# MarkTakken/kf2vecFSW

Measured on AMD Instinct MI355X. Metric: Gbases/s k-mer→.kf build at k=7; achieved HBM GB/s vs gfx950 peak, higher is better.
Workload: dtype u32

## Files before the change

include/kf2vec_gpu.h:

```cpp
#ifndef KF2VEC_GPU_H
#define KF2VEC_GPU_H

#include <stddef.h>
#include <stdint.h>

#ifdef __cplusplus
extern "C" {
#endif

#define KF_ABI_VERSION 1

#define KF_OK 0
#define KF_EINVAL (-1)
#define KF_EHIP (-2)
#define KF_ERANGE (-3)
#define KF_EFORMAT (-4)

#define KF_MIN_K 2
#define KF_MAX_K 12
#define KF_SPARSE_MAX_K 31

#define KF_ACCUMULATE 1u

#define KF_FMT_AUTO 0
// ... 12 lines not shown
int kf_index_records(const uint8_t* bytes, uint64_t len, int fmt, uint64_t base,
                     uint64_t* out_iv, uint64_t cap_pairs, uint64_t* n_pairs,
                     int* fmt_detected);

int kf_read_files(const char* const* paths, int32_t n, const uint64_t* sizes, const uint64_t* off,
                  uint8_t* dst, uint64_t piece, int n_threads);

int kf_index_fasta(const uint8_t* d_bytes, const uint64_t* d_goff, int32_t n_genomes,
                   uint64_t batch_bytes, uint64_t* d_excl, uint64_t cap_pairs,
                   uint64_t* d_n_pairs, uint32_t* d_scratch, uint64_t scratch_words, void* stream);

int kf_count_batch(const uint8_t* d_bytes, const uint64_t* d_goff, int32_t n_genomes,
                   const uint64_t* d_excl, uint64_t n_excl,
                   const uint32_t* d_code2col, const uint32_t* d_col2rep, int k,
                   uint32_t* d_counts, uint64_t* d_totals, uint32_t flags, void* stream);

int kf_workspace_reserve(int k, int32_t max_genomes);

int kf_count_launch_info(int k, int* grid, int* block, int* lds_bytes);

uint64_t kf_sparse_workspace_bytes(int k, uint64_t batch_bytes, int32_t n_genomes);
int kf_sparse_count(const uint8_t* d_bytes, const uint64_t* d_goff, int32_t n_genomes,
                    uint64_t batch_bytes, const uint64_t* d_excl, uint64_t n_excl, int k,
                    void* d_work, uint64_t work_bytes, uint64_t* d_keys, uint32_t* d_counts,
                    uint64_t* d_nuniq, void* stream);

const char* kf_build_id(void);

int kf_stream_probe(const uint8_t* d_bytes, uint64_t n, uint32_t* d_out, void* stream);

// ... 46 lines not shown
```

kf2vecfsw_amd/_native.py:

```python
from __future__ import annotations

import ctypes
import os

_HERE = os.path.dirname(os.path.abspath(__file__))
LIB_PATH = os.environ.get("KF2VEC_GPU_LIB") or os.path.join(_HERE, "libkf2vec_gpu.so")

KF_OK = 0
KF_EINVAL = -1
KF_EHIP = -2
KF_ERANGE = -3
KF_EFORMAT = -4
KF_MIN_K = 2
KF_MAX_K = 12
KF_SPARSE_MAX_K = 31
KF_ACCUMULATE = 1
KF_FMT_AUTO, KF_FMT_FASTA, KF_FMT_FASTQ = 0, 1, 2

_u64, _u32, _i32, _i64, _int = ctypes.c_uint64, ctypes.c_uint32, ctypes.c_int32, ctypes.c_int64, ctypes.c_int
_vp, _cp = ctypes.c_void_p, ctypes.c_char_p
_P64 = ctypes.POINTER(ctypes.c_uint64)
_PI = ctypes.POINTER(ctypes.c_int)
SIGNATURES = {
    "kf_abi_version": (_int, []),
    "kf_last_error": (_cp, []),
    "kf_num_bins": (_u64, [_int]),
    "kf_tables": (_int, [_int, _vp, _vp, _P64]),
    "kf_vocab_text": (_int, [_int, _vp, _u64, _P64]),
    "kf_index_records": (_int, [_vp, _u64, _int, _u64, _vp, _u64, _P64, _PI]),
    "kf_count_batch": (_int, [_vp, _vp, _i32, _vp, _u64, _vp, _vp, _int, _vp, _vp, _u32, _vp]),
    "kf_count_launch_info": (_int, [_int, _PI, _PI, _PI]),
    "kf_workspace_release": (_int, []),
    "kf_workspace_reserve": (_int, [_int, _i32]),
    "kf_build_id": (_cp, []),
    "kf_stream_probe": (_int, [_vp, _u64, _vp, _vp]),
    "kf_synth_fasta": (_int, [_vp, _vp, _i32, _i64, _i64, _u64, _u64, _int, _u64, _vp]),
    "kf_synth_genome_bytes": (_u64, [_i64, _u64, _int, _u64]),
    "kf_synth_header_len": (_u64, [_i64]),
    "kf_format_kf": (_int, [_cp, _vp, _u64, _int, _int, _vp, _u64, _P64]),
    "kf_write_kf_files": (_int, [_cp, ctypes.POINTER(_cp), _i32, _vp, _u64, _int, _int, _int]),
    "kf_write_kf_rows": (_int, [_cp, ctypes.POINTER(_cp), _i32, _vp, _u64, _int, _int, _int]),
    "kf_write_kf_segments": (_int, [_i32, ctypes.POINTER(_cp), _vp, _vp, ctypes.POINTER(_cp), ctypes.POINTER(_cp),
                                    _vp, _vp, _u32, _vp, _u64, _int, _int, _int]),
    "kf_write_kf_segments16": (_int, [_i32, ctypes.POINTER(_cp), _vp, _vp, ctypes.POINTER(_cp), ctypes.POINTER(_cp),
                                      _vp, _vp, _u32, _vp, _u64, _int, _int, _int]),
# ... 51 lines not shown
```

kf2vecfsw_amd/counter.py:

```python
from __future__ import annotations

import ctypes
import dataclasses
import os
from typing import Sequence

import numpy as np
import torch

from . import _native as N

ALIGN = 16


def num_bins(k: int) -> int:
    return int(N.lib().kf_num_bins(k))


def tables(k: int) -> tuple[np.ndarray, np.ndarray]:
    nb = num_bins(k)
    code2col = np.empty(1 << (2 * k), dtype=np.uint32)
    col2rep = np.empty(nb, dtype=np.uint32)
    n = ctypes.c_uint64(0)
    N.check(N.lib().kf_tables(k, code2col.ctypes.data, col2rep.ctypes.data, ctypes.byref(n)), "kf_tables")
# ... 153 lines not shown
                    raise N.NativeError(f"short read on {p}")
                got += r
        finally:
            os.close(fd)

    with ThreadPoolExecutor(max_workers=max(1, int(threads))) as ex:
        list(ex.map(read, jobs))
        excl = None
        if index:
            parts = list(ex.map(lambda i: index_records(d[int(off[i]): int(off[i]) + sizes[i]], N.KF_FMT_FASTA,
                                                        int(off[i]))[0], range(len(ranges))))
            excl = (np.concatenate(parts) if parts else np.zeros(0, np.uint64)).astype(np.uint64)
    return HostBatch(data, off, excl, list(names) if names else [f"{p}:{a}" for p, a, _ in ranges])


@dataclasses.dataclass
class DeviceBatch:
    data: torch.Tensor
    off: torch.Tensor
    excl: torch.Tensor
    n: int
    n_excl: int


def index_on_device(data: torch.Tensor, off: torch.Tensor, n: int, nbytes: int) -> tuple[torch.Tensor, int]:
    dev = data.device
    s = _stream_ptr(dev)
    nb = (nbytes + 4095) // 4096
    scratch = torch.empty(nb + 1, dtype=torch.int32, device=dev)
    npairs = torch.zeros(1, dtype=torch.int64, device=dev)
    cap = 64 * n + 4096
    while True:
        excl = torch.empty(max(2 * cap, 2), dtype=torch.int64, device=dev)
        N.check(N.lib().kf_index_fasta(data.data_ptr(), off.data_ptr(), n, nbytes, excl.data_ptr(), cap,
                                       npairs.data_ptr(), scratch.data_ptr(), nb + 1, s), "kf_index_fasta")
        m = int(npairs.item())
        if m <= cap:
            return excl[: 2 * m], m
        cap = m


def to_device(hb: HostBatch, device: torch.device | str = "cuda") -> DeviceBatch:
    dev = torch.device(device)
    if hb.dev_data is not None:
        cur = torch.cuda.current_stream(dev)
        if hb.dev_event is not None:
            cur.wait_event(hb.dev_event)
        data = hb.dev_data
        data.record_stream(cur)
    else:
        data = hb.data.to(dev, non_blocking=True)
    if hb.excl is None:
        pin = hb.data is None or hb.data.is_pinned()
        off = torch.from_numpy(hb.off.view(np.int64))
        off = (off.pin_memory() if pin else off).to(dev, non_blocking=pin)
        with torch.cuda.device(dev):
            excl, m = index_on_device(data, off, hb.n, int(hb.off[-1]))
        return DeviceBatch(data, off, excl if m else torch.zeros(2, dtype=torch.int64, device=dev), hb.n, m)
    ex = hb.excl if hb.excl.size else np.zeros(2, np.uint64)
    pin = hb.data is None or hb.data.is_pinned()
    n_off = (hb.off.size + 1) & ~1
    host = np.zeros(n_off + ex.size, np.int64)
    host[: hb.off.size] = hb.off.view(np.int64)
    host[n_off:] = ex.view(np.int64)
    small = torch.from_numpy(host)
    if pin:
        small = small.pin_memory()
    small = small.to(dev, non_blocking=pin)
    off, excl = small[: hb.off.size], small[n_off:]
    return DeviceBatch(data, off, excl, hb.n, hb.excl.size // 2)


def _stream_ptr(device: torch.device) -> int:
# ... 1 lines not shown


_DEV_TABLES: dict = {}


class KmerCounter:

    def __init__(self, k: int, device: torch.device | str = "cuda"):
        if not (N.KF_MIN_K <= k <= N.KF_MAX_K):
            raise ValueError(f"k={k} out of range [{N.KF_MIN_K}, {N.KF_MAX_K}]")
        self.k = k
        self.device = torch.device(device)
        if self.device.type != "cuda" or not torch.cuda.is_available():
            raise N.NativeError("KmerCounter needs a ROCm GPU (no CPU fallback)")
        self.nbins = num_bins(k)
        key = (k, self.device.index if self.device.index is not None else torch.cuda.current_device())
        if key not in _DEV_TABLES:
            c2c, c2r = tables(k)
            _DEV_TABLES[key] = (torch.from_numpy(c2c.view(np.int32)).to(self.device),
                                torch.from_numpy(c2r.view(np.int32)).to(self.device))
        self.code2col, self.col2rep = _DEV_TABLES[key]

    def launch_info(self) -> tuple[int, int, int]:
        g, b, l = ctypes.c_int(), ctypes.c_int(), ctypes.c_int()
        with torch.cuda.device(self.device):
            N.check(N.lib().kf_count_launch_info(self.k, ctypes.byref(g), ctypes.byref(b), ctypes.byref(l)),
                    "kf_count_launch_info")
        return g.value, b.value, l.value

    def reserve(self, max_genomes: int) -> None:
        with torch.cuda.device(self.device):
            N.check(N.lib().kf_workspace_reserve(self.k, int(max_genomes)), "kf_workspace_reserve")

    def alloc_out(self, n: int) -> tuple[torch.Tensor, torch.Tensor]:
        return (torch.empty((n, self.nbins), dtype=torch.int32, device=self.device),
                torch.empty(n, dtype=torch.int64, device=self.device))

    def count(self, db: DeviceBatch, counts: torch.Tensor | None = None, totals: torch.Tensor | None = None,
              accumulate: bool = False, stream: int | None = None) -> tuple[torch.Tensor, torch.Tensor]:
        if counts is None or totals is None:
            counts, totals = self.alloc_out(db.n)
        assert counts.shape == (db.n, self.nbins) and counts.dtype == torch.int32 and counts.is_contiguous()
        assert totals.shape == (db.n,) and totals.dtype == torch.int64
        assert db.data.data_ptr() % 16 == 0
        s = _stream_ptr(self.device) if stream is None else stream
        with torch.cuda.device(self.device):
            N.check(N.lib().kf_count_batch(
                db.data.data_ptr(), db.off.data_ptr(), db.n, db.excl.data_ptr() if db.n_excl else None,
                db.n_excl, self.code2col.data_ptr(), self.col2rep.data_ptr(), self.k,
                counts.data_ptr(), totals.data_ptr(), N.KF_ACCUMULATE if accumulate else 0, s), "kf_count_batch")
        return counts, totals


class SparseCounter:

    def __init__(self, k: int, device: torch.device | str = "cuda"):
        if not (N.KF_MIN_K <= k <= N.KF_SPARSE_MAX_K):
            raise ValueError(f"k={k} out of range [{N.KF_MIN_K}, {N.KF_SPARSE_MAX_K}]")
        self.k = k
        self.device = torch.device(device)
        if self.device.type != "cuda" or not torch.cuda.is_available():
            raise N.NativeError("SparseCounter needs a ROCm GPU (no CPU fallback)")
        self._work = None

    def workspace_bytes(self, batch_bytes: int, n: int) -> int:
# ... 104 lines not shown
```

kf2vecfsw_amd/csrc/kf_count.hip:

```cpp
#include <hip/hip_runtime.h>
#include <stdint.h>
#include <stdlib.h>

#include <mutex>

#include "kf_front.h"
#include "kf_internal.h"

namespace kf {

constexpr int kBlock = 1024;
#ifndef KF_WAVE_WEIGHTS
#define KF_WAVE_WEIGHTS (20u | 17u << 8 | 11u << 16 | 6u << 24)
#endif
constexpr uint32_t kWaveWeights = KF_WAVE_WEIGHTS;
constexpr int kXRing = 2;

__device__ __forceinline__ uint32_t lds_add_rtn(uint32_t a, uint32_t v) {
    return __hip_atomic_fetch_add((lds_u32*)(uintptr_t)a, v, __ATOMIC_RELAXED, __HIP_MEMORY_SCOPE_WORKGROUP);
}

__device__ __forceinline__ void lds_barrier() { asm volatile("s_waitcnt lgkmcnt(0)\n\ts_barrier" ::: "memory"); }

__device__ __forceinline__ void wg_span(const CountArgs& A, uint64_t& lo, uint64_t& hi) {
// ... 315 lines not shown
            uint32_t r[16];
            xc_wins8(*xs[i], r);
#pragma unroll
            for (int j = 0; j < 16; j += 4) o |= r[j] | r[j + 1] | r[j + 2] | r[j + 3];
        }
    }
    lane_total -= x0.nl + x1.nl + x2.nl;
    carry = tail_pack((uint32_t)__builtin_amdgcn_readlane((int)x2.c, kWave - 1) & TM, 31u, 31u);
    if (__builtin_amdgcn_ballot_w64((o & HOT) != 0) != 0) {
        x_scan_drain<K>(A.code2col, gcounts, lane);
        drained = 1;
    }
    return true;
}

template <int K, bool MASKED>
__device__ __forceinline__ uint32_t x_singles(const uint4 d, const CountArgs& A, uint64_t chunk, int lane,
                                              const ChunkMask& m, uint64_t iv0, uint32_t carry, uint32_t* gcounts,
                                              uint32_t& lane_total, uint32_t& drained) {
    constexpr uint32_t HOT = x_hot<K>();
    uint32_t C, V, EN, ne, own;
    front_end<K, MASKED, false>(d, A, chunk, lane, m, iv0, C, V, EN, ne, own);
    const Windows win = windows<K, MASKED>(C, V, EN, ne, carry, lane);
    const uint32_t wlo = win.wlo, whi = win.whi, R = win.R;
    if constexpr (K == 9) {
        drained |= k9b_region<false>(wlo, whi, R, A, gcounts);
        lane_total += (uint32_t)__builtin_popcount(R);
        return win.next;
    }
    const uint32_t wv[4] = {wlo, __builtin_amdgcn_alignbit(whi, wlo, 8), __builtin_amdgcn_alignbit(whi, wlo, 16),
                            __builtin_amdgcn_alignbit(whi, wlo, 24)};
    uint32_t o = 0;
#pragma unroll
    for (int r = 0; r < 16; ++r) {
        const int fo = (2 * r) & ~7;
        const uint32_t y = __builtin_amdgcn_ubfe(wv[fo >> 3], 2 * r - fo, 2 * K);
        o |= lds_add_rtn((K == 8 ? 0u : XL<K>::P) + ((y >> 1) << 2), ((R >> r) & 1u) * half_one(y));
    }
    if (__builtin_amdgcn_ballot_w64((o & HOT) != 0) != 0) {
        x_scan_drain<K>(A.code2col, gcounts, lane);
        drained = 1;
    }
    lane_total += (uint32_t)__builtin_popcount(R);
    return win.next;
}

template <int K>
__device__ __forceinline__ uint32_t x_range(const CountArgs& A, int32_t g, uint64_t glo, uint64_t ghi, uint64_t lo,
                                            uint64_t hi, int lane, uint32_t& drained) {
    if (lo >= hi) return 0;
    uint32_t* gcounts = A.counts + (uint64_t)g * A.nbins;
    Range rg;
    rg.init(glo, ghi, lo, hi);
    auto load = [&](uint32_t r) {
        return xc_load(A.bytes, rg.c0, r, rg.end_r, lane);
    };
    static_assert(kXRing == 2, "two-deep register ring");
    XBlock buf[K == 9 ? 1 : kXRing];
    XBlock b0, b1;
    if constexpr (K == 9) {
        b0 = load(0);
        b1 = load(kXChunk);
    } else {
#pragma unroll
        for (int j = 0; j < kXRing; ++j) buf[j] = load(j * kXChunk);
    }
    const uint32_t nx = (rg.nch + 2) / 3;
    rg.warm16<K>(A, lane);
    __builtin_amdgcn_s_setprio(0);
    uint32_t carry = rg.carry;
    uint32_t rel = 0;
    const ChunkMask m = rg.mask();
    uint32_t lane_total = 0;
    uint32_t nfast = 0;
    auto step = [&](const XBlock& bf) {
        bool fast = !rg.masked_span(A, rel, kXChunk);
        if (fast)
            fast = xc_fast<K>(bf, A, lane, carry, gcounts, lane_total, drained);
        nfast += fast ? 1u : 0u;
        if (!fast) {
            const bool m0 = rg.masked(A, rel);
            const uint64_t iv0 = rg.iv;
            const bool m1 = rg.masked(A, rel + kChunk);
            const uint64_t iv1 = rg.iv;
            const bool m2 = rg.masked(A, rel + 2 * kChunk);
#pragma unroll
            for (int h = 0; h < 3; ++h) {
                const uint32_t r = rel + h * kChunk;
                if (h > 0 && r >= rg.nch * kChunk) break;
                const bool mh = h == 0 ? m0 : (h == 1 ? m1 : m2);
                const uint64_t ivh = h == 0 ? iv0 : (h == 1 ? iv1 : rg.iv);
                const uint4 hb = bf.q[h];
                if (mh)
                    carry = x_singles<K, true>(hb, A, rg.c0 + r, lane, m, ivh, carry, gcounts, lane_total, drained);
                else
// ... 11 lines not shown
        }
        if (nx & 1u) step(b0);
    } else {
        for (uint32_t i = 0; i + kXRing <= nx; i += kXRing) {
#pragma unroll
            for (int j = 0; j < kXRing; ++j) {
                step(buf[j]);
                buf[j] = load(rel + (kXRing - 1) * kXChunk);
            }
        }
        const uint32_t rem = nx % kXRing;
#pragma unroll
        for (int j = 0; j < kXRing - 1; ++j)
            if (rem > (uint32_t)j) step(buf[j]);
    }
    return lane_total + 48u * nfast;
}

__device__ __forceinline__ uint32_t f_swz(uint32_t y) { return y ^ (((y >> 8) & 15u) << 1); }
__device__ __forceinline__ uint32_t u16sum2(uint32_t w) { return (w & 0xFFFFu) + (w >> 16); }

__device__ __forceinline__ void pair_f_sums(const uint32_t* hist, int tid, uint32_t (&F)[16]) {
    const uint4* h4 = (const uint4*)hist;
#pragma unroll
    for (int i = 0; i < 8; ++i) {
        const uint4 w = h4[i * 1024 + tid];
        F[2 * i] = u16sum2(w.x) + u16sum2(w.y);
        F[2 * i + 1] = u16sum2(w.z) + u16sum2(w.w);
#pragma unroll
        for (int a = 0; a < 4; ++a) {
// ... 11 lines not shown
#pragma unroll
    for (uint32_t m = 0; m < NM; ++m) {
        const uint32_t y = (uint32_t)tid + kBlock * m;
        F[m] = 0;
        if (y < NY) {
            const uint32_t sh = (y & 1u) << 4;
            uint32_t f = u16sum2(hist[2 * y]) + u16sum2(hist[2 * y + 1]);
#pragma unroll
            for (uint32_t a = 0; a < 4; ++a) f += (hist[a * (NY / 2) + (y >> 1)] >> sh) & 0xFFFFu;
            f += (hist[XL<K>::P / 4 + (y >> 1)] >> sh) & 0xFFFFu;
            F[m] = f;
        }
    }
}

template <int K>
__global__ void __launch_bounds__(kBlock) __attribute__((amdgpu_waves_per_eu(4, 4))) k1x_kernel(CountArgs A) {
    static_assert(K >= 2 && K <= 9, "K1x serves k = 2 .. 9 (k = 9: K9b byte counters)");
    extern __shared__ __attribute__((aligned(16))) uint32_t hist[];
    const int tid = threadIdx.x;
    const int lane = tid & (kWave - 1);
    const int wave = __builtin_amdgcn_readfirstlane(tid >> 6);
    {
        uint4* h4 = (uint4*)hist;
        for (uint32_t i = tid; i < XL<K>::bytes / 16; i += kBlock) h4[i] = make_uint4(0u, 0u, 0u, 0u);
    }
    __syncthreads();
    if ((uint32_t)(uintptr_t)(lds_u32*)hist != 0u) __builtin_trap();
    uint64_t span_lo, span_hi;
    wg_span(A, span_lo, span_hi);
    if (span_lo >= span_hi) return;
    int32_t g = (int32_t)wave_upper_bound((uint64_t)A.n_genomes, span_lo, lane,
                                          [&](uint64_t i) { return A.goff[i + 1]; });
    const uint32_t fr_lo = wave_frac((uint32_t)wave, kWaveWeights), fr_hi = wave_frac((uint32_t)wave + 1, kWaveWeights);
    for (; g < A.n_genomes; ++g) {
        __builtin_amdgcn_s_setprio(3);
        const uint64_t glo = A.goff[g], ghi = A.goff[g + 1];
        if (glo >= span_hi) break;
        const uint64_t plo = max(glo, span_lo), phi = min(ghi, span_hi);
        if (phi <= plo) continue;
        const uint64_t lo = split_at_frac(plo, phi, fr_lo), hi = split_at_frac(plo, phi, fr_hi);
        uint32_t drained = 0;
        unsigned long long s = x_range<K>(A, g, glo, ghi, lo, hi, lane, drained);
        uint32_t* gc = A.counts + (uint64_t)g * A.nbins;
        const bool whole = plo == glo && phi == ghi && !(A.flags & KF_ACCUMULATE);
        if constexpr (K == 9) {
            lds_barrier();
            if (lane == 0) hist[XL<K>::P / 4 + wave] = drained;
            lds_barrier();
            const uint4* fl = (const uint4*)(hist + XL<K>::P / 4);
            const uint4 f0 = fl[0], f1 = fl[1], f2 = fl[2], f3 = fl[3];
            const bool any_fix = (f0.x | f0.y | f0.z | f0.w | f1.x | f1.y | f1.z | f1.w | f2.x | f2.y | f2.z |
                                  f2.w | f3.x | f3.y | f3.z | f3.w) != 0;
            const uint8_t* hb = (const uint8_t*)hist;
            for (uint32_t c0 = (uint32_t)tid; c0 < (1u << 17); c0 += 4 * kBlock) {
                uint32_t rep[4];
#pragma unroll
                for (int j = 0; j < 4; ++j) rep[j] = A.col2rep[c0 + j * kBlock];
// ... 232 lines not shown
#pragma unroll
        for (int k = 0; k < 4; ++k)
#pragma unroll
            for (int q = 0; q < 3; ++q) acc ^= v[k][q].x ^ v[k][q].y ^ v[k][q].z ^ v[k][q].w;
    }
    acc = wave_xor(acc);
    if (lane == 0 && acc) atomicXor(out, acc);
}

}

using namespace kf;

namespace {

void* kernel_for(int k) {
    switch (k) {
    case 2: return (void*)&k1x_kernel<2>;
    case 3: return (void*)&k1x_kernel<3>;
    case 4: return (void*)&k1x_kernel<4>;
    case 5: return (void*)&k1x_kernel<5>;
    case 6: return (void*)&k1x_kernel<6>;
    case 7: return (void*)&k1x_kernel<7>;
    case 8: return (void*)&k1x_kernel<8>;
    case 9: return (void*)&k1x_kernel<9>;
    default: return nullptr;
    }
}

int lds_bytes_for(int k) {
    switch (k) {
    case 2: return (int)XL<2>::bytes;
    case 3: return (int)XL<3>::bytes;
    case 4: return (int)XL<4>::bytes;
    case 5: return (int)XL<5>::bytes;
    case 6: return (int)XL<6>::bytes;
    case 7: return (int)XL<7>::bytes;
    case 8: return (int)XL<8>::bytes;
    default: return (int)XL<9>::bytes;
    }
}


int g_grid[KF_MAX_K + 1][64];
std::mutex g_grid_mu;

int launch_info(int k, int* grid, int* block, int* lds) {
    int dev = 0;
    if (hipGetDevice(&dev) != hipSuccess) return kf_fail(KF_EHIP, "hipGetDevice failed");
    if (dev < 0 || dev >= 64) return kf_fail(KF_EINVAL, "device index out of range");
    const int l = lds_bytes_for(k);
    std::lock_guard<std::mutex> lk(g_grid_mu);
    int& gr = g_grid[k][dev];
    if (!gr) {
        void* fn = kernel_for(k);
        if (hipFuncSetAttribute(fn, hipFuncAttributeMaxDynamicSharedMemorySize, l) != hipSuccess)
            return kf_fail(KF_EHIP, "hipFuncSetAttribute(MaxDynamicSharedMemorySize) failed");
        int per_cu = 0, cus = 0;
        if (hipOccupancyMaxActiveBlocksPerMultiprocessor(&per_cu, fn, kBlock, l) != hipSuccess)
            return kf_fail(KF_EHIP, "hipOccupancyMaxActiveBlocksPerMultiprocessor failed");
        if (hipDeviceGetAttribute(&cus, hipDeviceAttributeMultiprocessorCount, dev) != hipSuccess)
            return kf_fail(KF_EHIP, "hipDeviceGetAttribute(MultiprocessorCount) failed");
        gr = (per_cu < 1 ? 1 : per_cu) * (cus > 0 ? cus : 1);
    }
    *grid = gr;
    *block = kBlock;
    *lds = l;
    return KF_OK;
}
}

extern "C" int kf_count_launch_info(int k, int* grid, int* block, int* lds_bytes) {
    if (k < KF_MIN_K || k > KF_MAX_K) return kf_fail(KF_EINVAL, "k out of range [2, 12]");
    if (!grid || !block || !lds_bytes) return kf_fail(KF_EINVAL, "null output pointer");
    if (k >= 10) return bucket_launch_info(k, grid, block, lds_bytes);
    return launch_info(k, grid, block, lds_bytes);
}

extern "C" int kf_workspace_reserve(int k, int32_t max_genomes) {
    if (k < KF_MIN_K || k > KF_MAX_K) return kf_fail(KF_EINVAL, "k out of range [2, 12]");
    if (max_genomes < 0) return kf_fail(KF_EINVAL, "max_genomes < 0");
    if (k >= 10) return bucket_reserve(k, max_genomes);
    int grid = 0, block = 0, lds = 0;
    return launch_info(k, &grid, &block, &lds);
}

extern "C" int kf_count_batch(const uint8_t* d_bytes, const uint64_t* d_goff, int32_t n_genomes,
                              const uint64_t* d_excl, uint64_t n_excl, const uint32_t* d_code2col,
                              const uint32_t* d_col2rep, int k, uint32_t* d_counts, uint64_t* d_totals,
                              uint32_t flags, void* stream) {
    if (k < KF_MIN_K || k > KF_MAX_K) return kf_fail(KF_EINVAL, "k out of range [2, 12]");
    if (n_genomes < 0) return kf_fail(KF_EINVAL, "n_genomes < 0");
    if (n_genomes == 0) return KF_OK;
    if (!d_bytes || !d_goff || !d_counts || !d_totals || !d_code2col || !d_col2rep)
        return kf_fail(KF_EINVAL, "null device pointer");
    if (n_excl && !d_excl) return kf_fail(KF_EINVAL, "d_excl is null but n_excl > 0");
    if (((uintptr_t)d_bytes) & 15) return kf_fail(KF_EINVAL, "d_bytes must be 16-byte aligned");
    const uint64_t nb = kf_num_bins(k);
    hipStream_t s = (hipStream_t)stream;
// ... 7 lines not shown
            hipMemsetAsync(d_totals, 0, (size_t)n_genomes * sizeof(uint64_t), s) != hipSuccess)
            return kf_fail(KF_EHIP, "hipMemsetAsync failed");
    }
    CountArgs A;
    A.bytes = d_bytes;
    A.goff = d_goff;
    A.excl = d_excl;
    A.n_excl = n_excl;
    A.code2col = d_code2col;
    A.col2rep = d_col2rep;
    A.counts = d_counts;
    A.totals = (unsigned long long*)d_totals;
    A.nbins = (uint32_t)nb;
    A.n_genomes = n_genomes;
    A.flags = flags;
    if (bucket) return bucket_launch(A, k, flags, s);
    int grid = 0, block = 0, lds = 0;
    const int rc = launch_info(k, &grid, &block, &lds);
    if (rc) return rc;

    void* args[] = {&A};
    if (hipLaunchKernel(kernel_for(k), dim3(grid), dim3(block), args, (size_t)lds, s) != hipSuccess)
        return kf_fail(KF_EHIP, "count kernel launch failed: %s", hipGetErrorString(hipGetLastError()));
    return KF_OK;
}

extern "C" int kf_stream_probe(const uint8_t* d_bytes, uint64_t n, uint32_t* d_out, void* stream) {
    if (!d_bytes || !d_out) return kf_fail(KF_EINVAL, "null device pointer");
    if (((uintptr_t)d_bytes) & 15) return kf_fail(KF_EINVAL, "d_bytes must be 16-byte aligned");
    if (n == 0) return KF_OK;
    int dev = 0, cus = 0;
    if (hipGetDevice(&dev) != hipSuccess ||
        hipDeviceGetAttribute(&cus, hipDeviceAttributeMultiprocessorCount, dev) != hipSuccess)
        return kf_fail(KF_EHIP, "device query failed");
    hipLaunchKernelGGL(stream_probe_kernel, dim3(2 * (cus > 0 ? cus : 1)), dim3(1024), 0, (hipStream_t)stream, d_bytes,
                       n, d_out);
    if (hipGetLastError() != hipSuccess) return kf_fail(KF_EHIP, "stream probe launch failed");
// ... 17 lines not shown
```

kf2vecfsw_amd/csrc/kf_front.h:

```cpp
#pragma once
#include <hip/hip_runtime.h>
#include <stdint.h>

namespace kf {

constexpr int kWave = 64;
constexpr int kChunk = 1024;

struct CountArgs {
    const uint8_t* bytes;
    const uint64_t* goff;
    const uint64_t* excl;
    uint64_t n_excl;
    const uint32_t* code2col;
    const uint32_t* col2rep;
    uint32_t* counts;
    unsigned long long* totals;
    uint32_t nbins;
    int32_t n_genomes;
    uint32_t flags;
};

__device__ __forceinline__ uint32_t tail_pack(uint32_t codes, uint32_t n, uint32_t ne) {
    return codes | (min(n, 31u) << 22) | (min(ne, 31u) << 27);
}
__device__ __forceinline__ uint32_t t_codes(uint32_t t) { return t & 0x3FFFFFu; }
__device__ __forceinline__ uint32_t t_n(uint32_t t) { return (t >> 22) & 31u; }
__device__ __forceinline__ uint32_t t_ne(uint32_t t) { return t >> 27; }

template <int K>
__device__ __forceinline__ uint32_t tail_combine(uint32_t a, uint32_t b) {
    constexpr uint32_t TM = (K > 1) ? ((1u << (2 * (K - 1))) - 1u) : 0u;
    const uint32_t bn = t_n(b), bne = t_ne(b);
    const uint32_t n = (bn < bne) ? bn : min(t_n(a) + bn, 31u);
    const uint32_t codes =
// ... 230 lines not shown
    uint32_t v = own;
#pragma unroll
    for (int dd = 1; dd < kWave; dd <<= 1) {
        const uint32_t o = __shfl_up(v, dd, kWave);
        if (lane >= dd) v = tail_combine<K>(o, v);
    }
    return (uint32_t)__builtin_amdgcn_readlane((int)v, kWave - 1);
}

template <int K>
__device__ __forceinline__ uint32_t chunk_tail(const uint8_t* bytes, const uint64_t* excl, uint64_t n_excl, int64_t p,
                                               uint64_t glo, int lane) {
    return chunk_tail_data<K>(chunk_tail_load(bytes, p, glo, lane), bytes, excl, n_excl, p, glo, lane);
}


struct Range {
    uint64_t c0, glo, ghi, lo, hi;
    uint32_t lo_r, hi_r, end_r, nch;
    uint64_t iv;
    uint32_t ivs_r, ive_r;
    uint64_t ivs_a, ive_a;
    uint32_t carry;

    __device__ __forceinline__ uint32_t rel_of(uint64_t x) const {
        return x <= c0 ? 0u : (x - c0 >= 0xFFFFFFFFull ? 0xFFFFFFFFu : (uint32_t)(x - c0));
    }
    __device__ __forceinline__ void init(uint64_t glo_, uint64_t ghi_, uint64_t lo_, uint64_t hi_) {
        glo = glo_, ghi = ghi_, lo = lo_, hi = hi_;
        c0 = lo & ~(uint64_t)15;
// ... 161 lines not shown
```

kf2vecfsw_amd/main.py:

```python
from __future__ import annotations

import argparse
import ctypes
import multiprocessing as mp
import os
import sys
from concurrent.futures import ThreadPoolExecutor

import numpy as np

from . import _native as N

__version__ = "kf2vec 0.1.3 (kf2vecfsw_amd MI355X)"

default_k_len = 7
min_k_len = 2
max_k_len = 31
supported_k = range(3, 12)

FORMATS = [".fq", ".fastq", ".fa", ".fna", ".fasta"]
_SUFFIXES = tuple(FORMATS)


def list_inputs(input_dir: str) -> tuple[list[str], list[str]]:
# ... 190 lines not shown
    if not os.path.exists(args.output_dir):
        print("No such directory '{}'".format(args.output_dir), file=sys.stderr)
        sys.exit(0)

    files_names, samples_names = list_inputs(args.input_dir)
    if shard is not None:
        sizes = [os.path.getsize(os.path.join(args.input_dir, f)) for f in files_names]
        mine = shard_files(sizes, samples_names, shard[1])[shard[0]]
        files_names = [files_names[i] for i in mine]
        samples_names = [samples_names[i] for i in mine]
    if args.k not in supported_k:
        raise ValueError("k={} has no vocabulary: supported k are {}..{}".format(
            args.k, supported_k.start, supported_k.stop - 1))

    import torch
    from .counter import KmerCounter, pack_files, to_device

    if shard is not None and not os.environ.get("KF_SHARD"):
        _join_group()
    dflt = f"cuda:{os.environ.get('LOCAL_RANK', '0')}" if shard is not None else "cuda"
    device = torch.device(getattr(args, "device", None) or dflt)
    if not files_names:
        _finish(args, shard, lead)
        return
    counter = KmerCounter(args.k, device)
    paths = [os.path.join(args.input_dir, f) for f in files_names]
    batch_gb = getattr(args, "batch_gb", None)
    fsz = [os.path.getsize(p) for p in paths]
    asz = [(x + 15) // 16 * 16 for x in fsz]
    batches = _size_batches(fsz, _pipeline_budget(paths, batch_gb, fsz), ramp=True,
                            max_files=_count_cap(4 * counter.nbins, batch_gb))
# ... 38 lines not shown
    writer = ThreadPoolExecutor(max_workers=1)
    ahead = n_slots
    reads = deque(reader.submit(pack, i, batches[i]) for i in range(min(ahead, len(batches))))
    big = slot_bytes
    with torch.cuda.stream(copy_stream):
        warm = torch.empty(big + 16, dtype=torch.uint8, device=device)
        warm[:16].zero_()
        del warm
    with torch.cuda.stream(stream):
        torch.cuda.Event(enable_timing=True).record(stream)
    copy_stream.synchronize()
    stream.synchronize()
    writes = []
    behind = max(1, int(os.environ.get("KF_WRITE_BEHIND", "2")))

    def write(ev, host, names):
        ev.synchronize()
        t0 = now_ms()
        c = host.numpy().view(np.uint32)
        write_kf_files(args.output_dir, names, c, args.pseudocount, args.raw_cnt, threads)
        if trace:
            tr.append(("write", names[0] if names else "", t0, now_ms()))

    evs = []
    for bi, idx in enumerate(batches):
        t_wait = now_ms()
        hb = reads.popleft().result()
        if trace:
            tr.append(("got", bi, t_wait, now_ms()))
        if bi + ahead < len(batches):
            reads.append(reader.submit(pack, bi + ahead, batches[bi + ahead]))
        with torch.cuda.stream(stream):
            if trace:
                e = [torch.cuda.Event(enable_timing=True) for _ in range(4)]
                e[0].record(stream)
                evs.append((bi, now_ms(), e))
            db = to_device(hb, device)
            del hb
            if trace:
                e[1].record(stream)
                th = [now_ms()]
            counts, _ = counter.count(db, stream=stream.cuda_stream)
            if trace:
                e[2].record(stream)
                th.append(now_ms())
            keep = [j for j, i in enumerate(idx) if last[samples_names[i]] == i]
            rows = counts if len(keep) == len(idx) else counts[torch.tensor(keep, device=device)]
            host = torch.empty(rows.shape, dtype=rows.dtype, pin_memory=True)
            if trace:
                th.append(now_ms())
            host.copy_(rows, non_blocking=True)
            ev = torch.cuda.Event()
            ev.record(stream)
            if trace:
                e[3].record(stream)
                th.append(now_ms())
        for i in idx:
            if args.pseudocount:
                print(">>> Adding pseudocounts. Sample: {}".format(files_names[i]))
            if not args.raw_cnt:
                print(">>> Normalizing. Sample: {}".format(files_names[i]))
        if bi >= behind:
            writes[bi - behind].result()
        writes.append(writer.submit(write, ev, host, [samples_names[idx[j]] for j in keep]))
        del host, rows, counts, db
        if trace:
            th.append(now_ms())
            tr.append(("issue", bi, th))
    for w in writes:
        w.result()
    t_written = now_ms()
    reader.shutdown()
    writer.shutdown()
    files_pool.shutdown()
    if trace and evs:
        base_cpu = evs[0][1]
        e00 = evs[0][2][0]
        for bi, t_issue, e in evs:
            d = [round(base_cpu + e00.elapsed_time(x), 3) for x in e]
# ... 550 lines not shown
```

Measured before the change: 5751.

## Fuse FASTA header detection into the k-mer count kernel for k up to 9

After: 5752, median of 3. About the same (+0.0%).

```diff
diff --git a/include/kf2vec_gpu.h b/include/kf2vec_gpu.h
--- a/include/kf2vec_gpu.h
+++ b/include/kf2vec_gpu.h
@@ -50,6 +50,11 @@
                    const uint64_t* d_excl, uint64_t n_excl,
                    const uint32_t* d_code2col, const uint32_t* d_col2rep, int k,
                    uint32_t* d_counts, uint64_t* d_totals, uint32_t flags, void* stream);
+
+int kf_count_batch_fasta(const uint8_t* d_bytes, const uint64_t* d_goff, int32_t n_genomes,
+                         const uint32_t* d_code2col, const uint32_t* d_col2rep, int k,
+                         uint32_t* d_counts, uint64_t* d_totals, uint32_t* d_status,
+                         uint32_t flags, void* stream);
 
 int kf_workspace_reserve(int k, int32_t max_genomes);
 
diff --git a/kf2vecfsw_amd/_native.py b/kf2vecfsw_amd/_native.py
--- a/kf2vecfsw_amd/_native.py
+++ b/kf2vecfsw_amd/_native.py
@@ -29,6 +29,7 @@
     "kf_vocab_text": (_int, [_int, _vp, _u64, _P64]),
     "kf_index_records": (_int, [_vp, _u64, _int, _u64, _vp, _u64, _P64, _PI]),
     "kf_count_batch": (_int, [_vp, _vp, _i32, _vp, _u64, _vp, _vp, _int, _vp, _vp, _u32, _vp]),
+    "kf_count_batch_fasta": (_int, [_vp, _vp, _i32, _vp, _vp, _int, _vp, _vp, _vp, _u32, _vp]),
     "kf_count_launch_info": (_int, [_int, _PI, _PI, _PI]),
     "kf_workspace_release": (_int, []),
     "kf_workspace_reserve": (_int, [_int, _i32]),
diff --git a/kf2vecfsw_amd/counter.py b/kf2vecfsw_amd/counter.py
--- a/kf2vecfsw_amd/counter.py
+++ b/kf2vecfsw_amd/counter.py
@@ -191,13 +191,18 @@
     return HostBatch(data, off, excl, list(names) if names else [f"{p}:{a}" for p, a, _ in ranges])
 
 
+FUSED_MAX_K = 9
+
+
 @dataclasses.dataclass
 class DeviceBatch:
     data: torch.Tensor
     off: torch.Tensor
-    excl: torch.Tensor
+    excl: torch.Tensor | None
     n: int
     n_excl: int
+    indexed: bool = True
+    nbytes: int = 0
 
 
 def index_on_device(data: torch.Tensor, off: torch.Tensor, n: int, nbytes: int) -> tuple[torch.Tensor, int]:
@@ -217,7 +222,17 @@
         cap = m
 
 
-def to_device(hb: HostBatch, device: torch.device | str = "cuda") -> DeviceBatch:
+def index_batch(db: DeviceBatch) -> DeviceBatch:
+    if db.indexed:
+        return db
+    dev = db.data.device
+    with torch.cuda.device(dev):
+        excl, m = index_on_device(db.data, db.off, db.n, db.nbytes)
+    return DeviceBatch(db.data, db.off, excl if m else torch.zeros(2, dtype=torch.int64, device=dev), db.n, m,
+                       True, db.nbytes)
+
+
+def to_device(hb: HostBatch, device: torch.device | str = "cuda", index: bool = True) -> DeviceBatch:
     dev = torch.device(device)
     if hb.dev_data is not None:
         cur = torch.cuda.current_stream(dev)
@@ -231,9 +246,8 @@
         pin = hb.data is None or hb.data.is_pinned()
         off = torch.from_numpy(hb.off.view(np.int64))
         off = (off.pin_memory() if pin else off).to(dev, non_blocking=pin)
-        with torch.cuda.device(dev):
-            excl, m = index_on_device(data, off, hb.n, int(hb.off[-1]))
-        return DeviceBatch(data, off, excl if m else torch.zeros(2, dtype=torch.int64, device=dev), hb.n, m)
+        db = DeviceBatch(data, off, None, hb.n, 0, False, int(hb.off[-1]))
+        return index_batch(db) if index else db
     ex = hb.excl if hb.excl.size else np.zeros(2, np.uint64)
     pin = hb.data is None or hb.data.is_pinned()
     n_off = (hb.off.size + 1) & ~1
@@ -265,7 +279,8 @@
         if self.device.type != "cuda" or not torch.cuda.is_available():
             raise N.NativeError("KmerCounter needs a ROCm GPU (no CPU fallback)")
         self.nbins = num_bins(k)
-        key = (k, self.device.index if self.device.index is not None else torch.cuda.current_device())
+        self.status = None
+        key =(k, self.device.index if self.device.index is not None else torch.cuda.current_device())
         if key not in _DEV_TABLES:
             c2c, c2r = tables(k)
             _DEV_TABLES[key] = (torch.from_numpy(c2c.view(np.int32)).to(self.device),
@@ -288,7 +303,17 @@
                 torch.empty(n, dtype=torch.int64, device=self.device))
 
     def count(self, db: DeviceBatch, counts: torch.Tensor | None = None, totals: torch.Tensor | None = None,
-              accumulate: bool = False, stream: int | None = None) -> tuple[torch.Tensor, torch.Tensor]:
+              accumulate: bool = False, stream: int | None = None,
+              status: torch.Tensor | None = None) -> tuple[torch.Tensor, torch.Tensor]:
+        self.status = None
+        if not db.indexed:
+            if self.k > FUSED_MAX_K:
+                db = index_batch(db)
+            else:
+                return self._count_fused(db, counts, totals, accumulate, stream, status)
+        return self._count_indexed(db, counts, totals, accumulate, stream)
+
+    def _count_indexed(self, db, counts=None, totals=None, accumulate=False, stream=None):
         if counts is None or totals is None:
             counts, totals = self.alloc_out(db.n)
         assert counts.shape == (db.n, self.nbins) and counts.dtype == torch.int32 and counts.is_contiguous()
@@ -300,6 +325,35 @@
                 db.data.data_ptr(), db.off.data_ptr(), db.n, db.excl.data_ptr() if db.n_excl else None,
                 db.n_excl, self.code2col.data_ptr(), self.col2rep.data_ptr(), self.k,
                 counts.data_ptr(), totals.data_ptr(), N.KF_ACCUMULATE if accumulate else 0, s), "kf_count_batch")
+        return counts, totals
+
+    def recount_indexed(self, db: DeviceBatch) -> tuple[torch.Tensor, torch.Tensor]:
+        return self._count_indexed(index_batch(db))
+
+    def _count_fused(self, db, counts, totals, accumulate, stream, status):
+        if counts is None or totals is None:
+            counts = torch.empty((db.n, self.nbins), dtype=torch.int32, device=self.device)
+            tot = torch.empty(db.n + 1, dtype=torch.int64, device=self.device)
+            totals, status = tot[: db.n], tot[db.n:].view(torch.int32)[:1]
+        elif status is None:
+            status = torch.zeros(1, dtype=torch.int32, device=self.device)
+        assert counts.shape == (db.n, self.nbins) and counts.dtype == torch.int32 and counts.is_contiguous()
+        assert totals.shape == (db.n,) and totals.dtype == torch.int64
+        assert status.shape == (1,) and status.dtype == torch.int32
+        assert db.data.data_ptr() % 16 == 0
+        s = _stream_ptr(self.device) if stream is None else stream
+        with torch.cuda.device(self.device):
+            N.check(N.lib().kf_count_batch_fasta(
+                db.data.data_ptr(), db.off.data_ptr(), db.n, self.code2col.data_ptr(), self.col2rep.data_ptr(),
+                self.k, counts.data_ptr(), totals.data_ptr(), status.data_ptr(),
+                N.KF_ACCUMULATE if accumulate else 0, s), "kf_count_batch_fasta")
+        self.status = status
+        return counts, totals
+
+    def count_checked(self, db: DeviceBatch) -> tuple[torch.Tensor, torch.Tensor]:
+        counts, totals = self.count(db)
+        if self.status is not None and int(self.status.item()) != 0:
+            counts, totals = self.recount_indexed(db)
         return counts, totals
 
 
diff --git a/kf2vecfsw_amd/csrc/kf_count.hip b/kf2vecfsw_amd/csrc/kf_count.hip
--- a/kf2vecfsw_amd/csrc/kf_count.hip
+++ b/kf2vecfsw_amd/csrc/kf_count.hip
@@ -353,13 +353,25 @@
     return true;
 }
 
-template <int K, bool MASKED>
+template <int K, bool MASKED, bool HDR = false>
 __device__ __forceinline__ uint32_t x_singles(const uint4 d, const CountArgs& A, uint64_t chunk, int lane,
                                               const ChunkMask& m, uint64_t iv0, uint32_t carry, uint32_t* gcounts,
-                                              uint32_t& lane_total, uint32_t& drained) {
+                                              uint32_t& lane_total, uint32_t& drained, uint32_t hm = 0) {
     constexpr uint32_t HOT = x_hot<K>();
     uint32_t C, V, EN, ne, own;
-    front_end<K, MASKED, false>(d, A, chunk, lane, m, iv0, C, V, EN, ne, own);
+    if constexpr (HDR) {
+        static_assert(MASKED, "the header-aware chunk is always masked");
+        uint32_t INV, NNL;
+        classify16(d, C, INV, NNL);
+        const int64_t b0 = (int64_t)(chunk + 16u * (uint32_t)lane);
+        INV |= range_bits(-1, (int64_t)m.glo - b0) | hm;
+        EN = range_bits((int64_t)m.lo - b0, (int64_t)m.hi - b0);
+        V = ~INV & 0xFFFFu;
+        ne = (uint32_t)__builtin_popcount(NNL);
+        compact<true>(NNL ^ 0xFFFFu, C, V, EN);
+    } else {
+        front_end<K, MASKED, false>(d, A, chunk, lane, m, iv0, C, V, EN, ne, own);
+    }
     const Windows win = windows<K, MASKED>(C, V, EN, ne, carry, lane);
     const uint32_t wlo = win.wlo, whi = win.whi, R = win.R;
     if constexpr (K == 9) {
@@ -384,7 +396,7 @@
     return win.next;
 }
 
-template <int K>
+template <int K, bool HDR>
 __device__ __forceinline__ uint32_t x_range(const CountArgs& A, int32_t g, uint64_t glo, uint64_t ghi, uint64_t lo,
                                             uint64_t hi, int lane, uint32_t& drained) {
     if (lo >= hi) return 0;
@@ -405,7 +417,16 @@
         for (int j = 0; j < kXRing; ++j) buf[j] = load(j * kXChunk);
     }
     const uint32_t nx = (rg.nch + 2) / 3;
-    rg.warm16<K>(A, lane);
+    HdrState hs{0u, 0u, 0ull};
+    uint32_t longh = 0;
+    (void)hs, (void)longh;
+    if constexpr (HDR) {
+        const HdrWarm hw = hdr_warm<K>(A.bytes, rg.c0, glo, ghi, lane);
+        rg.carry = rfl(hw.carry);
+        hs = hdr_state(hw.st.in_hdr, hw.st.pnl, (uint32_t)hw.st.hstart, (uint32_t)(hw.st.hstart >> 32));
+    } else {
+        rg.warm16<K>(A, lane);
+    }
     __builtin_amdgcn_s_setprio(0);
     uint32_t carry = rg.carry;
     uint32_t rel = 0;
@@ -413,11 +434,31 @@
     uint32_t lane_total = 0;
     uint32_t nfast = 0;
     auto step = [&](const XBlock& bf) {
-        bool fast = !rg.masked_span(A, rel, kXChunk);
+        bool fast;
+        if constexpr (HDR)
+            fast = !hs.in_hdr && !(rel < rg.lo_r || rel + kXChunk > rg.hi_r);
+        else
+            fast = !rg.masked_span(A, rel, kXChunk);
         if (fast)
             fast = xc_fast<K>(bf, A, lane, carry, gcounts, lane_total, drained);
         nfast += fast ? 1u : 0u;
-        if (!fast) {
+        if constexpr (HDR) {
+            if (fast) {
+                hs.pnl = ((uint32_t)__builtin_amdgcn_readlane((int)bf.q[2].w, kWave - 1) >> 24) == (uint32_t)'\n';
+            } else {
+#pragma unroll
+                for (int h = 0; h < 3; ++h) {
+                    const uint32_t r = rel + h * kChunk;
+                    if (h > 0 && r >= rg.nch * kChunk) break;
+                    const HdrChunk hc =
+                        hdr_chunk(bf.q[h], (int64_t)(rg.c0 + r), glo, ghi, lane, hs.in_hdr, hs.pnl, hs.hstart);
+                    carry = x_singles<K, true, true>(bf.q[h], A, rg.c0 + r, lane, m, 0, carry, gcounts, lane_total,
+                                                     drained, hc.H);
+                    hs = hc.state();
+                    longh |= rfl(hc.longh);
+                }
+            }
+        } else if (!fast) {
             const bool m0 = rg.masked(A, rel);
             const uint64_t iv0 = rg.iv;
             const bool m1 = rg.masked(A, rel + kChunk);
@@ -459,6 +500,9 @@
         for (int j = 0; j < kXRing - 1; ++j)
             if (rem > (uint32_t)j) step(buf[j]);
     }
+    if constexpr (HDR) {
+        if (longh && lane == 0) atomicOr(A.status, 1u);
+    }
     return lane_total + 48u * nfast;
 }
 
@@ -500,7 +544,7 @@
     }
 }
 
-template <int K>
+template <int K, bool HDR = false>
 __global__ void __launch_bounds__(kBlock) __attribute__((amdgpu_waves_per_eu(4, 4))) k1x_kernel(CountArgs A) {
     static_assert(K >= 2 && K <= 9, "K1x serves k = 2 .. 9 (k = 9: K9b byte counters)");
     extern __shared__ __attribute__((aligned(16))) uint32_t hist[];
@@ -527,7 +571,7 @@
         if (phi <= plo) continue;
         const uint64_t lo = split_at_frac(plo, phi, fr_lo), hi = split_at_frac(plo, phi, fr_hi);
         uint32_t drained = 0;
-        unsigned long long s = x_range<K>(A, g, glo, ghi, lo, hi, lane, drained);
+        unsigned long long s = x_range<K, HDR>(A, g, glo, ghi, lo, hi, lane, drained);
         uint32_t* gc = A.counts + (uint64_t)g * A.nbins;
         const bool whole = plo == glo && phi == ghi && !(A.flags & KF_ACCUMULATE);
         if constexpr (K == 9) {
@@ -790,7 +834,20 @@
 
 namespace {
 
-void* kernel_for(int k) {
+void* kernel_for(int k, bool hdr = false) {
+    if (hdr) {
+        switch (k) {
+        case 2: return (void*)&k1x_kernel<2, true>;
+        case 3: return (void*)&k1x_kernel<3, true>;
+        case 4: return (void*)&k1x_kernel<4, true>;
+        case 5: return (void*)&k1x_kernel<5, true>;
+        case 6: return (void*)&k1x_kernel<6, true>;
+        case 7: return (void*)&k1x_kernel<7, true>;
+        case 8: return (void*)&k1x_kernel<8, true>;
+        case 9: return (void*)&k1x_kernel<9, true>;
+        default: return nullptr;
+        }
+    }
     switch (k) {
     case 2: return (void*)&k1x_kernel<2>;
     case 3: return (void*)&k1x_kernel<3>;
@@ -818,18 +875,18 @@
 }
 
 
-int g_grid[KF_MAX_K + 1][64];
+int g_grid[2][KF_MAX_K + 1][64];
 std::mutex g_grid_mu;
 
-int launch_info(int k, int* grid, int* block, int* lds) {
+int launch_info(int k, int* grid, int* block, int* lds, bool hdr = false) {
     int dev = 0;
     if (hipGetDevice(&dev) != hipSuccess) return kf_fail(KF_EHIP, "hipGetDevice failed");
     if (dev < 0 || dev >= 64) return kf_fail(KF_EINVAL, "device index out of range");
     const int l = lds_bytes_for(k);
     std::lock_guard<std::mutex> lk(g_grid_mu);
-    int& gr = g_grid[k][dev];
+    int& gr = g_grid[hdr ? 1 : 0][k][dev];
     if (!gr) {
-        void* fn = kernel_for(k);
+        void* fn = kernel_for(k, hdr);
         if (hipFuncSetAttribute(fn, hipFuncAttributeMaxDynamicSharedMemorySize, l) != hipSuccess)
             return kf_fail(KF_EHIP, "hipFuncSetAttribute(MaxDynamicSharedMemorySize) failed");
         int per_cu = 0, cus = 0;
@@ -858,7 +915,8 @@
     if (max_genomes < 0) return kf_fail(KF_EINVAL, "max_genomes < 0");
     if (k >= 10) return bucket_reserve(k, max_genomes);
     int grid = 0, block = 0, lds = 0;
-    return launch_info(k, &grid, &block, &lds);
+    const int rc = launch_info(k, &grid, &block, &lds);
+    return rc ? rc : launch_info(k, &grid, &block, &lds, true);
 }
 
 extern "C" int kf_count_batch(const uint8_t* d_bytes, const uint64_t* d_goff, int32_t n_genomes,
@@ -896,6 +954,7 @@
     A.nbins = (uint32_t)nb;
     A.n_genomes = n_genomes;
     A.flags = flags;
+    A.status = nullptr;
     if (bucket) return bucket_launch(A, k, flags, s);
     int grid = 0, block = 0, lds = 0;
     const int rc = launch_info(k, &grid, &block, &lds);
@@ -903,6 +962,54 @@
 
     void* args[] = {&A};
     if (hipLaunchKernel(kernel_for(k), dim3(grid), dim3(block), args, (size_t)lds, s) != hipSuccess)
+        return kf_fail(KF_EHIP, "count kernel launch failed: %s", hipGetErrorString(hipGetLastError()));
+    return KF_OK;
+}
+
+extern "C" int kf_count_batch_fasta(const uint8_t* d_bytes, const uint64_t* d_goff, int32_t n_genomes,
+                                    const uint32_t* d_code2col, const uint32_t* d_col2rep, int k,
+                                    uint32_t* d_counts, uint64_t* d_totals, uint32_t* d_status, uint32_t flags,
+                                    void* stream) {
+    if (k < KF_MIN_K || k > KF_MAX_K) return kf_fail(KF_EINVAL, "k out of range [2, 12]");
+    if (k >= 10)
+        return kf_fail(KF_EINVAL, "kf_count_batch_fasta serves k = 2..9 (k = %d: kf_index_fasta + kf_count_batch)", k);
+    if (n_genomes < 0) return kf_fail(KF_EINVAL, "n_genomes < 0");
+    if (!d_status) return kf_fail(KF_EINVAL, "null device pointer (d_status)");
+    hipStream_t s = (hipStream_t)stream;
+    if (n_genomes == 0) {
+        if (!(flags & KF_ACCUMULATE) && hipMemsetAsync(d_status, 0, sizeof(uint32_t), s) != hipSuccess)
+            return kf_fail(KF_EHIP, "hipMemsetAsync failed");
+        return KF_OK;
+    }
+    if (!d_bytes || !d_goff || !d_counts || !d_totals || !d_code2col || !d_col2rep)
+        return kf_fail(KF_EINVAL, "null device pointer");
+    if (((uintptr_t)d_bytes) & 15) return kf_fail(KF_EINVAL, "d_bytes must be 16-byte aligned");
+    const uint64_t nb = kf_num_bins(k);
+    if (!(flags & KF_ACCUMULATE)) {
+        const bool after = (const void*)d_status == (const void*)(d_totals + n_genomes);
+        if (hipMemsetAsync(d_counts, 0, (size_t)n_genomes * nb * sizeof(uint32_t), s) != hipSuccess ||
+            hipMemsetAsync(d_totals, 0, ((size_t)n_genomes + (after ? 1 : 0)) * sizeof(uint64_t), s) != hipSuccess ||
+            (!after && hipMemsetAsync(d_status, 0, sizeof(uint32_t), s) != hipSuccess))
+            return kf_fail(KF_EHIP, "hipMemsetAsync failed");
+    }
+    CountArgs A;
+    A.bytes = d_bytes;
+    A.goff = d_goff;
+    A.excl = nullptr;
+    A.n_excl = 0;
+    A.code2col = d_code2col;
+    A.col2rep = d_col2rep;
+    A.counts = d_counts;
+    A.totals = (unsigned long long*)d_totals;
+    A.nbins = (uint32_t)nb;
+    A.n_genomes = n_genomes;
+    A.flags = flags;
+    A.status = d_status;
+    int grid = 0, block = 0, lds = 0;
+    const int rc = launch_info(k, &grid, &block, &lds, true);
+    if (rc) return rc;
+    void* args[] = {&A};
+    if (hipLaunchKernel(kernel_for(k, true), dim3(grid), dim3(block), args, (size_t)lds, s) != hipSuccess)
         return kf_fail(KF_EHIP, "count kernel launch failed: %s", hipGetErrorString(hipGetLastError()));
     return KF_OK;
 }
diff --git a/kf2vecfsw_amd/csrc/kf_front.h b/kf2vecfsw_amd/csrc/kf_front.h
--- a/kf2vecfsw_amd/csrc/kf_front.h
+++ b/kf2vecfsw_amd/csrc/kf_front.h
@@ -19,6 +19,7 @@
     uint32_t nbins;
     int32_t n_genomes;
     uint32_t flags;
+    uint32_t* status;
 };
 
 __device__ __forceinline__ uint32_t tail_pack(uint32_t codes, uint32_t n, uint32_t ne) {
@@ -279,6 +280,124 @@
     return chunk_tail_data<K>(chunk_tail_load(bytes, p, glo, lane), bytes, excl, n_excl, p, glo, lane);
 }
 
+constexpr uint32_t kHdrLong = kChunk;
+
+struct HdrState {
+    uint32_t in_hdr, pnl;
+    uint64_t hstart;
+};
+__device__ __forceinline__ uint32_t rfl(uint32_t v) { return (uint32_t)__builtin_amdgcn_readfirstlane((int)v); }
+__device__ __forceinline__ HdrState hdr_state(uint32_t in_hdr, uint32_t pnl, uint32_t hs_lo, uint32_t hs_hi) {
+    return HdrState{rfl(in_hdr), rfl(pnl), ((uint64_t)rfl(hs_hi) << 32) | (uint64_t)rfl(hs_lo)};
+}
+struct HdrChunk {
+    uint32_t H, in_hdr, pnl, hs_lo, hs_hi, longh;
+    __device__ __forceinline__ HdrState state() const { return hdr_state(in_hdr, pnl, hs_lo, hs_hi); }
+};
+
+__device__ inline __noinline__ HdrChunk hdr_chunk(const uint4 d, int64_t chunk, uint64_t glo, uint64_t ghi, int lane,
+                                           uint32_t in_hdr, uint32_t pnl, uint64_t hstart) {
+    in_hdr = __builtin_amdgcn_readfirstlane(in_hdr);
+    const int64_t b0 = chunk + 16 * lane;
+    const int64_t ga = (int64_t)glo - b0, gb = (int64_t)ghi - b0;
+    const uint32_t a = ga < 0 ? 0u : (ga > 16 ? 16u : (uint32_t)ga), b = gb < 0 ? 0u : (gb > 16 ? 16u : (uint32_t)gb);
+    const uint32_t pm = b > a ? (((1u << b) - 1u) & ~((1u << a) - 1u)) : 0u;
+    const uint32_t w[4] = {d.x, d.y, d.z, d.w};
+    uint32_t GT = 0, NL = 0;
+#pragma unroll
+    for (int i = 0; i < 16; ++i) {
+        const uint32_t c = (w[i >> 2] >> (8 * (i & 3))) & 0xFFu;
+        GT |= (c == (uint32_t)'>' ? 1u : 0u) << i;
+        NL |= (c == (uint32_t)'\n' ? 1u : 0u) << i;
+    }
+    GT &= pm;
+    NL &= pm;
+    uint32_t LS = ((NL << 1) | wave_shr1(pnl, NL >> 15)) & 0xFFFFu;
+    if (ga >= 0 && ga < 16) LS |= 1u << (uint32_t)ga;
+    const uint32_t HS = GT & LS;
+    const uint64_t evb = __ballot((HS | NL) != 0u), outb = __ballot(HS > NL);
+    const uint64_t below = evb & ((1ull << lane) - 1ull);
+    uint32_t s = below ? (uint32_t)((outb >> (63 - __builtin_clzll(below))) & 1ull) : in_hdr;
+    uint32_t H = 0;
+#pragma unroll
+    for (int i = 0; i < 16; ++i) {
+        s = (s | (HS >> i)) & ~(NL >> i) & 1u;
+        H |= s << i;
+    }
+    HdrChunk r;
+    r.H = __builtin_bitreverse32(H) >> 16;
+    r.longh = 0;
+    if (in_hdr) {
+        const uint64_t nlb = __ballot(NL != 0u);
+        if (nlb) {
+            const int l0 = __builtin_ctzll(nlb);
+            const int64_t e = chunk + 16 * l0 + __builtin_ctz((uint32_t)__shfl((int)NL, l0, kWave));
+            if ((uint64_t)e - hstart >= (uint64_t)kHdrLong) r.longh = 1;
+        }
+    }
+    const uint64_t hsb = __ballot(HS != 0u);
+    if (hsb) {
+        const int l1 = 63 - __builtin_clzll(hsb);
+        hstart = (uint64_t)(chunk + 16 * l1 + 31 - __builtin_clz((uint32_t)__shfl((int)HS, l1, kWave)));
+    }
+    r.in_hdr = evb ? (uint32_t)((outb >> (63 - __builtin_clzll(evb))) & 1ull) : in_hdr;
+    if (r.in_hdr) {
+        const uint64_t endp = min((uint64_t)(chunk + kChunk), ghi);
+        if (endp - hstart >= (uint64_t)kHdrLong) r.longh = 1;
+    }
+    r.pnl = (uint32_t)__builtin_amdgcn_readlane((int)(NL >> 15), kWave - 1);
+    r.hs_lo = (uint32_t)hstart;
+    r.hs_hi = (uint32_t)(hstart >> 32);
+    return r;
+}
+
+template <int K>
+__device__ __noinline__ uint32_t hdr_chunk_tail(const uint4 d, int64_t p, uint64_t glo, int lane, uint32_t hm) {
+    uint32_t C, INV, NNL;
+    classify16(d, C, INV, NNL);
+    INV |= range_bits(-1, (int64_t)glo - (p + 16 * lane)) | hm;
+    uint32_t V = ~INV & 0xFFFFu, EN = 0;
+    const uint32_t ne = (uint32_t)__builtin_popcount(NNL);
+    compact<false>(NNL ^ 0xFFFFu, C, V, EN);
+    uint32_t v = own_tail<K>(C, V, ne);
+#pragma unroll
+    for (int dd = 1; dd < kWave; dd <<= 1) {
+        const uint32_t o = __shfl_up(v, dd, kWave);
+        if (lane >= dd) v = tail_combine<K>(o, v);
+    }
+    return (uint32_t)__builtin_amdgcn_readlane((int)v, kWave - 1);
+}
+
+struct HdrWarm {
+    uint32_t carry;
+    HdrState st;
+};
+template <int K>
+__device__ __noinline__ HdrWarm hdr_warm(const uint8_t* bytes, uint64_t c0, uint64_t glo, uint64_t ghi, int lane) {
+    HdrWarm w{tail_pack(0, 0, 0), HdrState{0u, 0u, 0ull}};
+    if (c0 <= glo) return w;
+    for (int64_t n = 1;; ++n) {
+        const int64_t ps = (int64_t)c0 - n * kChunk;
+        HdrState st{0u, 0u, 0ull};
+        if (ps > (int64_t)glo)
+            st = hdr_chunk(chunk_tail_load(bytes, ps - kChunk, glo, lane), ps - kChunk, glo, ghi, lane, 0u, 0u, 0ull)
+                     .state();
+        uint32_t t = tail_pack(0, 0, 0);
+        for (int64_t q = ps; q < (int64_t)c0; q += kChunk) {
+            const uint4 d = chunk_tail_load(bytes, q, glo, lane);
+            const HdrChunk h = hdr_chunk(d, q, glo, ghi, lane, st.in_hdr, st.pnl, st.hstart);
+            t = tail_combine<K>(t, hdr_chunk_tail<K>(d, q, glo, lane, h.H));
+            st = h.state();
+        }
+        t = __builtin_amdgcn_readfirstlane(t);
+        if (ps <= (int64_t)glo || tail_complete<K>(t)) {
+            w.carry = t;
+            w.st = st;
+            return w;
+        }
+    }
+}
+
 
 struct Range {
     uint64_t c0, glo, ghi, lo, hi;
diff --git a/kf2vecfsw_amd/main.py b/kf2vecfsw_amd/main.py
--- a/kf2vecfsw_amd/main.py
+++ b/kf2vecfsw_amd/main.py
@@ -228,7 +228,7 @@
             args.k, supported_k.start, supported_k.stop - 1))
 
     import torch
-    from .counter import KmerCounter, pack_files, to_device
+    from .counter import FUSED_MAX_K, KmerCounter, pack_files, to_device
 
     if shard is not None and not os.environ.get("KF_SHARD"):
         _join_group()
@@ -297,9 +297,19 @@
     writes = []
     behind = max(1, int(os.environ.get("KF_WRITE_BEHIND", "2")))
 
-    def write(ev, host, names):
+    fb_stream = torch.cuda.Stream(device)
+
+    def write(ev, host, names, hstat=None, db=None, keep=None):
         ev.synchronize()
         t0 = now_ms()
+        if hstat is not None and int(hstat[0]) != 0:
+            with torch.cuda.stream(fb_stream):
+                db.data.record_stream(fb_stream)
+                counts, _ = counter.recount_indexed(db)
+                rows = counts if len(keep) == db.n else counts[torch.tensor(keep, device=device)]
+                host.copy_(rows)
+            fb_stream.synchronize()
+        del db
         c = host.numpy().view(np.uint32)
         write_kf_files(args.output_dir, names, c, args.pseudocount, args.raw_cnt, threads)
         if trace:
@@ -318,7 +328,7 @@
                 e = [torch.cuda.Event(enable_timing=True) for _ in range(4)]
                 e[0].record(stream)
                 evs.append((bi, now_ms(), e))
-            db = to_device(hb, device)
+            db = to_device(hb, device, index=args.k > FUSED_MAX_K)
             del hb
             if trace:
                 e[1].record(stream)
@@ -333,6 +343,10 @@
             if trace:
                 th.append(now_ms())
             host.copy_(rows, non_blocking=True)
+            hstat = None
+            if counter.status is not None:
+                hstat = torch.empty(1, dtype=torch.int32, pin_memory=True)
+                hstat.copy_(counter.status, non_blocking=True)
             ev = torch.cuda.Event()
             ev.record(stream)
             if trace:
@@ -345,7 +359,8 @@
                 print(">>> Normalizing. Sample: {}".format(files_names[i]))
         if bi >= behind:
             writes[bi - behind].result()
-        writes.append(writer.submit(write, ev, host, [samples_names[idx[j]] for j in keep]))
+        writes.append(writer.submit(write, ev, host, [samples_names[idx[j]] for j in keep], hstat,
+                                    db if hstat is not None else None, keep))
         del host, rows, counts, db
         if trace:
             th.append(now_ms())
```
